# arendu-zz/MacaronicUserModeling

Hardware: AMD Instinct MI355X
Metric: LBP sweep iters/sec (whole node), batch=8192 graphs |X|=64 (higher is better)
Workload: dtype f64

## Files before the change

### macaronicusermodeling_amd/csrc/mlbp_lean.hip

```cpp
#include <hip/hip_runtime.h>

#include <vector>

#include "mlbp_device.h"
#include "mlbp_internal.h"

using mlbp::fail;
using namespace mlbp_dev;

namespace {

constexpr int WG = 256;

typedef double nt_d2 __attribute__((ext_vector_type(2)));
#define NT_LOAD2(p) ([&] { const nt_d2 v_ = __builtin_nontemporal_load(reinterpret_cast<const nt_d2*>(p)); return make_double2(v_.x, v_.y); }())

constexpr int UOP_VAR = 1;
constexpr int UOP_MT = 2;
constexpr int UOP_PSLOT_SHIFT = 2;
constexpr int UOP_NOP = 32;
constexpr int UOP_STORE_VF = 64;
constexpr int UOP_NSRC_SHIFT = 8;
constexpr int UOP_CARRY_IN = 0x1000;
constexpr int UOP_CARRY_OUT = 0x2000;
constexpr int GROUP_WORDS = 48;

struct LeanDev {
  const int32_t* image;
  const int32_t* readout;
  uint8_t* bail;
  int32_t n_bundles, HL, n_cprod, WL, n_ext, init, dense, keep;
};

__device__ __forceinline__ double swapadd16(double a, double b) {
  auto lo = __builtin_amdgcn_permlane16_swap((unsigned)__double2loint(a), (unsigned)__double2loint(b), false, false);
  auto hi = __builtin_amdgcn_permlane16_swap((unsigned)__double2hiint(a), (unsigned)__double2hiint(b), false, false);
  return __hiloint2double((int)hi[0], (int)lo[0]) + __hiloint2double((int)hi[1], (int)lo[1]);
}
__device__ __forceinline__ double swapadd32(double a, double b) {
  auto lo = __builtin_amdgcn_permlane32_swap((unsigned)__double2loint(a), (unsigned)__double2loint(b), false, false);
  auto hi = __builtin_amdgcn_permlane32_swap((unsigned)__double2hiint(a), (unsigned)__double2hiint(b), false, false);
  return __hiloint2double((int)hi[0], (int)lo[0]) + __hiloint2double((int)hi[1], (int)lo[1]);
}

__device__ __forceinline__ bool vote_any(bool p, int32_t* votes, int wave, int lane) {
  const int mine = __ballot(p) != 0 ? 1 : 0;
  if (lane == 0) votes[wave] = mine;
  lds_barrier();
  const int4 v = *reinterpret_cast<const int4*>(votes);
  return (v.x | v.y | v.z | v.w) != 0;
}

struct LaneGeo {
  int tm0, tm1;
  int mt;
  int red_tm;
  int red_mt;
  bool up, st_tm, st_mt, wr_tm;
};

__device__ __forceinline__ double2 lds2(const char* p) { return *reinterpret_cast<const double2*>(p); }
__device__ __forceinline__ void mul2(double2& a, const double2 b) { a.x *= b.x; a.y *= b.y; }

struct RegTable {
  const double2 (&T)[4][2];
  __device__ __forceinline__ double2 operator()(int r, int k) const { return T[r][k]; }
};
struct LdsTable {
  const double2* base;
  __device__ __forceinline__ double2 operator()(int r, int k) const { return base[(r * 2 + k) * WG]; }
};

template <bool MT, typename TB>
__device__ __forceinline__ void contract(const TB T, char* wb, int u0, int s1, int s2, int s3, int s4, int vf,
                                         const LaneGeo& G, char* redA) {
  const int nsrc = (u0 >> UOP_NSRC_SHIFT) & 15;
  const bool has_vf = (u0 & UOP_STORE_VF) != 0;
  if (MT) {
    double2 ma = lds2(wb + s1 + G.mt), mb = lds2(wb + s1 + G.mt + 16);
    if (nsrc > 1) {
      const double2 a = lds2(wb + s2 + G.mt), b = lds2(wb + s2 + G.mt + 16);
      mul2(ma, a); mul2(mb, b);
      if (nsrc > 2) {
        const double2 a2 = lds2(wb + s3 + G.mt), b2 = lds2(wb + s3 + G.mt + 16);
        mul2(ma, a2); mul2(mb, b2);
        if (nsrc > 3) { const double2 a3 = lds2(wb + s4 + G.mt), b3 = lds2(wb + s4 + G.mt + 16); mul2(ma, a3); mul2(mb, b3); }
      }
    }
    if (has_vf && G.st_mt) {
      *reinterpret_cast<double2*>(wb + vf + G.mt) = ma;
      *reinterpret_cast<double2*>(wb + vf + G.mt + 16) = mb;
    }
    double a00, a01, a10, a11;
    { const double2 t0 = T(0, 0), t1 = T(0, 1); a00 = ma.x * t0.x; a01 = ma.x * t0.y; a10 = ma.x * t1.x; a11 = ma.x * t1.y; }
    { const double2 t0 = T(1, 0), t1 = T(1, 1); a00 += ma.y * t0.x; a01 += ma.y * t0.y; a10 += ma.y * t1.x; a11 += ma.y * t1.y; }
    { const double2 t0 = T(2, 0), t1 = T(2, 1); a00 += mb.x * t0.x; a01 += mb.x * t0.y; a10 += mb.x * t1.x; a11 += mb.x * t1.y; }
    { const double2 t0 = T(3, 0), t1 = T(3, 1); a00 += mb.y * t0.x; a01 += mb.y * t0.y; a10 += mb.y * t1.x; a11 += mb.y * t1.y; }
    a00 += dpp_mov<0x128>(a10);
    a01 += dpp_mov<0x128>(a11);
    *reinterpret_cast<double*>(redA + G.red_mt) = swapadd32(a00, a01);
  } else {
    double2 m0 = lds2(wb + s1 + G.tm0), m1 = lds2(wb + s1 + G.tm1);
    if (nsrc > 1) {
      const double2 a = lds2(wb + s2 + G.tm0), b = lds2(wb + s2 + G.tm1);
      mul2(m0, a); mul2(m1, b);
      if (nsrc > 2) {
        const double2 a2 = lds2(wb + s3 + G.tm0), b2 = lds2(wb + s3 + G.tm1);
        mul2(m0, a2); mul2(m1, b2);
        if (nsrc > 3) { const double2 a3 = lds2(wb + s4 + G.tm0), b3 = lds2(wb + s4 + G.tm1); mul2(m0, a3); mul2(m1, b3); }
      }
    }
    if (has_vf && G.st_tm) {
      *reinterpret_cast<double2*>(wb + vf + G.tm0) = m0;
      *reinterpret_cast<double2*>(wb + vf + G.tm1) = m1;
    }
    double v[4];
#pragma unroll
    for (int r = 0; r < 4; ++r) {
      const double2 t0 = T(r, 0), t1 = T(r, 1);
      v[r] = t0.x * m0.x;
      v[r] += t0.y * m0.y;
      v[r] += t1.x * m1.x;
      v[r] += t1.y * m1.y;
    }
    const double u0 = swapadd16(v[0], v[2]), u1 = swapadd16(v[1], v[3]);
    const double keep = G.up ? u1 : u0, send = G.up ? u0 : u1;
    double w = keep + dpp_mov<0x141>(send);
    w += dpp_mov<0xB1>(w);
    w += dpp_mov<0x4E>(w);
    *reinterpret_cast<double*>(redA + G.red_tm) = w;
  }
}

template <int NT, int NL>
__device__ __forceinline__ void front(const double2 (&tab)[NT][4][2], const double2* tl, char* wb, int u0, const int4& lo, const int4& hi,
                                      const LaneGeo& G, char* redA) {
  const int pslot = (u0 >> UOP_PSLOT_SHIFT) & 7;
#pragma unroll
  for (int p = 0; p < NT; ++p) {
    if (p == pslot) {
      if (u0 & UOP_MT) contract<true>(RegTable{tab[p]}, wb, u0, lo.y, lo.z, lo.w, hi.x, hi.y, G, redA);
      else contract<false>(RegTable{tab[p]}, wb, u0, lo.y, lo.z, lo.w, hi.x, hi.y, G, redA);
    }
  }
  if (NL > 0 && pslot >= NT) {
    const LdsTable T = {tl + (size_t)(pslot - NT) * 8 * WG};
    if (u0 & UOP_MT) contract<true>(T, wb, u0, lo.y, lo.z, lo.w, hi.x, hi.y, G, redA);
    else contract<false>(T, wb, u0, lo.y, lo.z, lo.w, hi.x, hi.y, G, redA);
  }
}

template <int NT>
__device__ __forceinline__ void gradient_epilogue(const SweepDev& d, const GradFusedDev& gf, const double2 (&tab)[NT][4][2],
                                                  const char* wb, const int32_t* gst, double* scratch, const LaneGeo& G, int g,
                                                  int R_, int c_, int b3_) {
  constexpr int FEE = 3, FED = 6;
  const int t = threadIdx.x, lane = t & 63, wave = __builtin_amdgcn_readfirstlane(t >> 6);
  double lf[FEE] = {0.0, 0.0, 0.0};
  bool lbad = false;
  if (t < NT && t < d.P) {
    const int l0 = gf.pair_label[((size_t)g * d.P + t) * 2], l1 = gf.pair_label[((size_t)g * d.P + t) * 2 + 1];
    if ((unsigned)l0 >= 64u || (unsigned)l1 >= 64u) lbad = true;
    else {
      const double* phl = (gf.pair_phi[t] ? gf.phi_en_en_w1 : gf.phi_en_en) + ((size_t)l0 * 64 + l1) * FEE;
#pragma unroll
      for (int q = 0; q < FEE; ++q) lf[q] = phl[q];
    }
  }
  int which = 0;
  double2 W[NT][4][2];
  double* zs = scratch + 512;
  double* lfs = scratch + 544;
#pragma unroll
  for (int p = 0; p < NT; ++p) {
    double z = 0.0;
    if (p < d.P) {
      const int cs = as_const(gf.pair_c_slot)[p], rs = as_const(gf.pair_r_slot)[p];
      which |= (as_const(gf.pair_phi)[p] ? 1 : 0) << p;
      const double2 ca = lds2(wb + cs * 512 + G.mt), cb = lds2(wb + cs * 512 + G.mt + 16);
      const double2 r0 = lds2(wb + rs * 512 + G.tm0), r1 = lds2(wb + rs * 512 + G.tm1);
#pragma unroll
      for (int r = 0; r < 4; ++r) {
        const double ci = r == 0 ? ca.x : (r == 1 ? ca.y : (r == 2 ? cb.x : cb.y));
#pragma unroll
        for (int k = 0; k < 2; ++k) {
          const double2 rj = k ? r1 : r0, T = tab[p][r][k];
          W[p][r][k] = make_double2((ci * rj.x) * T.x, (ci * rj.y) * T.y);
          z += W[p][r][k].x + W[p][r][k].y;
        }
      }
      z = wave_sum(z);
      if (lane == 0) zs[wave * NT + p] = z;
    } else {
#pragma unroll
      for (int r = 0; r < 4; ++r) W[p][r][0] = W[p][r][1] = make_double2(0.0, 0.0);
    }
  }
  if (lbad) atomicExch(d.status, 1);
  if (t < NT && t < d.P) {
#pragma unroll
    for (int q = 0; q < FEE; ++q) lfs[t * FEE + q] = lf[q];
  }
  lds_barrier();
  double2 V[2][4][2];
#pragma unroll
  for (int tz = 0; tz < 2; ++tz)
#pragma unroll
    for (int r = 0; r < 4; ++r) V[tz][r][0] = V[tz][r][1] = make_double2(0.0, 0.0);
#pragma unroll
  for (int p = 0; p < NT; ++p) {
    if (p < d.P) {
      const double Z = (zs[p] + zs[NT + p]) + (zs[2 * NT + p] + zs[3 * NT + p]);
      const double inv = Z > 0.0 ? 1.0 / Z : 0.0;
      const double i0 = ((which >> p) & 1) ? 0.0 : inv, i1 = ((which >> p) & 1) ? inv : 0.0;
#pragma unroll
      for (int r = 0; r < 4; ++r)
#pragma unroll
        for (int k = 0; k < 2; ++k) {
          V[0][r][k].x += W[p][r][k].x * i0; V[0][r][k].y += W[p][r][k].y * i0;
          V[1][r][k].x += W[p][r][k].x * i1; V[1][r][k].y += W[p][r][k].y * i1;
        }
    }
  }
  double gacc[2][FEE] = {{0.0, 0.0, 0.0}, {0.0, 0.0, 0.0}};
  const int all = (1 << (d.P < NT ? d.P : NT)) - 1;
#pragma unroll
  for (int tz = 0; tz < 2; ++tz) {
    if (tz ? (which & all) == 0 : (which & all) == all) continue;
    typedef double v2d __attribute__((ext_vector_type(2)));
    typedef const v2d __attribute__((address_space(1))) * gptr2;
    const double* phi = tz ? gf.phi_en_en_w1 : gf.phi_en_en;
#pragma unroll
    for (int k = 0; k < 2; ++k) {
      const int col = 32 * (k ? 1 - b3_ : b3_) + 2 * c_;
      v2d cell[4][3];
#pragma unroll
      for (int r = 0; r < 4; ++r) {
        const gptr2 ph = (gptr2)(uintptr_t)(phi + ((size_t)(4 * R_ + r) * 64 + col) * FEE);
        cell[r][0] = ph[0]; cell[r][1] = ph[1]; cell[r][2] = ph[2];
      }
#pragma unroll
      for (int r = 0; r < 4; ++r) {
        const double w0 = V[tz][r][k].x, w1 = V[tz][r][k].y;
        gacc[tz][0] += w0 * cell[r][0].x + w1 * cell[r][1].y;
        gacc[tz][1] += w0 * cell[r][0].y + w1 * cell[r][2].x;
        gacc[tz][2] += w0 * cell[r][1].x + w1 * cell[r][2].y;
      }
    }
  }
  double gsum[FEE];
#pragma unroll
  for (int q = 0; q < FEE; ++q) gsum[q] = wave_sum(gacc[0][q] + gacc[1][q]);
  double lab_ee[FEE] = {0.0, 0.0, 0.0}, lab_ed[FED] = {0.0, 0.0, 0.0, 0.0, 0.0, 0.0};
  double exp_ee[FEE] = {0.0, 0.0, 0.0}, exp_ed[FED] = {0.0, 0.0, 0.0, 0.0, 0.0, 0.0};
  bool bad = false;
  constexpr int UB = 6;
  const int U = d.U;
  for (int u0 = wave; u0 < U; u0 += 4 * UB) {
    double b[UB], pv[UB][FED];
    int kd[UB], at[UB];
#pragma unroll
    for (int j = 0; j < UB; ++j) {
      const int u = u0 + 4 * j;
      kd[j] = -1;
      if (u < U) {
        const int kind = __builtin_amdgcn_readfirstlane(gst[2 * U + u]), obs = __builtin_amdgcn_readfirstlane(gst[3 * U + u]);
        const int lab = __builtin_amdgcn_readfirstlane(gst[4 * U + u]);
        const int cols = kind == 2 ? gf.Vde : 64;
        if ((unsigned)obs >= (unsigned)cols || (unsigned)lab >= 64u || (unsigned)kind > 2u) { bad = true; continue; }
        kd[j] = kind;
        const int slot = __builtin_amdgcn_readfirstlane(gst[u]);
        b[j] = __builtin_amdgcn_readfirstlane(gst[U + u]) ? *reinterpret_cast<const double*>(wb + slot * 512 + lane * 8) : 0.0;
        if (kind == 2) {
          const double2* ph = reinterpret_cast<const double2*>(gf.phi_en_de_t + ((size_t)obs * 64 + lane) * FED);
          at[j] = (obs * 64 + lab) * FED;
          const double2 a0 = ph[0], a1 = ph[1], a2 = ph[2];
          pv[j][0] = a0.x; pv[j][1] = a0.y; pv[j][2] = a1.x; pv[j][3] = a1.y; pv[j][4] = a2.x; pv[j][5] = a2.y;
        } else {
          typedef const double __attribute__((address_space(1))) * gptr1;
          const gptr1 ph = (gptr1)(uintptr_t)((kind ? gf.phi_en_en_w1_t : gf.phi_en_en_t) + ((size_t)obs * 64 + lane) * FEE);
          at[j] = (obs * 64 + lab) * FEE;
#pragma unroll
          for (int q = 0; q < FEE; ++q) pv[j][q] = ph[q];
        }
      }
    }
#pragma unroll
    for (int j = 0; j < UB; ++j) {
      if (kd[j] == 2) {
#pragma unroll
        for (int q = 0; q < FED; ++q) { lab_ed[q] += as_const_f64(gf.phi_en_de_t)[at[j] + q]; exp_ed[q] += b[j] * pv[j][q]; }
      } else if (kd[j] >= 0) {
        const double* base = kd[j] ? gf.phi_en_en_w1_t : gf.phi_en_en_t;
#pragma unroll
        for (int q = 0; q < FEE; ++q) { lab_ee[q] += as_const_f64(base)[at[j] + q]; exp_ee[q] += b[j] * pv[j][q]; }
      }
    }
  }
  if (bad && lane == 0) atomicExch(d.status, 1);
  constexpr int PER = FEE + FEE + FED;
  {
    double ue[FEE], ud[FED];
#pragma unroll
    for (int q = 0; q < FEE; ++q) ue[q] = lab_ee[q] - wave_sum(exp_ee[q]);
#pragma unroll
    for (int q = 0; q < FED; ++q) ud[q] = lab_ed[q] - wave_sum(exp_ed[q]);
    if (lane == 0) {
      double* o = scratch + wave * PER;
#pragma unroll
      for (int q = 0; q < FEE; ++q) o[q] = gsum[q];
#pragma unroll
      for (int q = 0; q < FEE; ++q) o[FEE + q] = ue[q];
#pragma unroll
      for (int q = 0; q < FED; ++q) o[FEE + FEE + q] = ud[q];
    }
  }
  lds_barrier();
  if (t == 0) {
    double tot[PER];
#pragma unroll
    for (int q = 0; q < PER; ++q) tot[q] = (scratch[q] + scratch[PER + q]) + (scratch[2 * PER + q] + scratch[3 * PER + q]);
    double gee[FEE];
#pragma unroll
    for (int q = 0; q < FEE; ++q) gee[q] = tot[FEE + q] - tot[q];
#pragma unroll
    for (int p = 0; p < NT; ++p) {
      if (p < d.P) {
#pragma unroll
        for (int q = 0; q < FEE; ++q) gee[q] += lfs[p * FEE + q];
      }
    }
#pragma unroll
    for (int q = 0; q < FEE; ++q) gf.grad_en_en[(size_t)g * FEE + q] = gee[q];
#pragma unroll
    for (int q = 0; q < FED; ++q) gf.grad_en_de[(size_t)g * FED + q] = tot[FEE + FEE + q];
  }
}

__device__ __forceinline__ double rescale(double r, int& bad) {
  const unsigned key = mag_key(r);
  const unsigned long long normal = __ballot(key - KEY_MIN < KEY_BAD - KEY_MIN);
  const unsigned long long wrong = __ballot(key >= KEY_BAD);
  bad |= (wrong != 0) | (normal == 0);
  const int ref = __builtin_amdgcn_readlane((int)key, normal ? __builtin_ctzll(normal) : 0);
  return __builtin_ldexp(r, 1023 - ((ref >> 20) & 0x7FF));
}

template <int NT, bool PADX, bool MULTI, int NL, bool GRAD>
__global__ __launch_bounds__(WG, (NT >= 7 ? 1 : (NT >= 4 ? 2 : 3))) void sweep_x64_lean_kernel(SweepDev d, LeanDev f, const int32_t* groups,
                                                                                             int n_groups, GradFusedDev gf) {
  int g = blockIdx.x;
  if (MULTI) {
    int lo = 0, hi = n_groups - 1;
    while (lo < hi) {
      const int mid = (lo + hi + 1) >> 1;
      if (as_const(groups)[(size_t)mid * GROUP_WORDS] <= g) lo = mid; else hi = mid - 1;
    }
    const int32_t* G = groups + (size_t)lo * GROUP_WORDS;
    const Words16 w0 = sload16(G), w1 = sload16(G + 16), w2 = sload16(G + 32);
    auto ptr = [](int32_t a, int32_t b) { return (uintptr_t)(uint32_t)a | ((uintptr_t)(uint32_t)b << 32); };
    g -= w0.w[0];
    f.image = (const int32_t*)ptr(w0.w[2], w0.w[3]); f.readout = (const int32_t*)ptr(w0.w[4], w0.w[5]);
    f.bail = (uint8_t*)ptr(w0.w[6], w0.w[7]); d.msgs = (double*)ptr(w0.w[8], w0.w[9]);
    d.marginals = (double*)ptr(w0.w[10], w0.w[11]); d.pair_tables = (const double*)ptr(w0.w[12], w0.w[13]);
    d.pair_tab = (const int32_t*)ptr(w0.w[14], w0.w[15]); d.unary_tables = (const double*)ptr(w1.w[0], w1.w[1]);
    d.unary_tab = (const int32_t*)ptr(w1.w[2], w1.w[3]); d.status = (int32_t*)ptr(w1.w[4], w1.w[5]);
    f.n_bundles = w1.w[6]; f.HL = w1.w[7]; f.n_cprod = w1.w[8]; f.WL = w1.w[9]; f.n_ext = w1.w[10];
    d.n_msgs = w1.w[11]; d.P = w1.w[12]; d.U = w1.w[13]; d.n_vars = w1.w[14]; d.n_pair_tables = w1.w[15];
    d.n_unary_tables = w2.w[0]; f.dense = w2.w[1];
  }
  extern __shared__ double lds[];
  double* work = lds;
  double* red = lds + (size_t)(d.n_msgs + f.n_ext) * 64;
  int32_t* limg = reinterpret_cast<int32_t*>(red + 4 * 256);
  double2* tl = reinterpret_cast<double2*>(limg + 16 * (f.n_bundles + 1));
  int32_t* gst = reinterpret_cast<int32_t*>(tl + (size_t)NL * 8 * WG);

  const int t = threadIdx.x, lane = t & 63, wave = __builtin_amdgcn_readfirstlane(t >> 6);
  const int X = PADX ? d.X : 64;
  const double uniform = 1.0 / (double)X;
  const double uni_l = (!PADX || lane < X) ? uniform : 0.0;
  double* gm = d.msgs + (size_t)g * d.n_msgs * X;
  const int32_t* img_hoist = f.image + 16 * (size_t)f.n_bundles;
  const int32_t* img_cprod = img_hoist + 8 * (size_t)f.HL;
  const int32_t* img_written = img_cprod + 16 * (size_t)f.n_cprod;
  int32_t* votes = reinterpret_cast<int32_t*>(red);
  constexpr bool LEAN_SYNC = !GRAD;

  LaneGeo G;
  const int c_ = (lane & 7) | ((lane >> 1) & 8), b3_ = (lane >> 3) & 1, R_ = 4 * wave + (b3_ | ((lane >> 5) << 1));
  {
    const int b5 = lane >> 5, b4 = (lane >> 4) & 1, b2 = (lane >> 2) & 1;
    G.tm0 = (32 * b3_ + 2 * c_) * 8;
    G.tm1 = (32 * (1 - b3_) + 2 * c_) * 8;
    G.mt = 4 * R_ * 8;
    G.red_tm = (4 * R_ + 2 * b4 + b2) * 8;
    G.red_mt = (wave * 64 + 32 * b3_ + 2 * c_ + b5) * 8;
    G.up = b2 != 0;
    G.st_tm = wave == 0 && (lane & 0x28) == 0;
    G.st_mt = (lane & 0x17) == 0;
    G.wr_tm = (lane & 3) == 0;
  }

  if (t == 0) f.bail[g] = 0;
  int g_kind = 0, g_obs = 0, g_lab = 0;
  if (GRAD && t < d.U) {
    g_kind = gf.unary_kind[t]; g_obs = gf.unary_obs[(size_t)g * d.U + t]; g_lab = gf.unary_label[(size_t)g * d.U + t];
  }
  bool ok = true;
  constexpr int HB = 8;
  double ur[HB];
  int uslot[HB], ufac[HB];
  {
    const Words16 hl = sload16(img_hoist + wave * 2 * f.HL);
#pragma unroll
    for (int j = 0; j < HB; ++j) {
      const int u = hl.w[2 * j];
      uslot[j] = hl.w[2 * j + 1];
      ufac[j] = u;
      ur[j] = 0.0;
      if (u >= 0) {
        const int row = f.dense ? g * d.U + u : as_const(d.unary_tab)[(size_t)g * d.U + u];
        if ((unsigned)row >= (unsigned)d.n_unary_tables) ok = false;
        else if (!PADX || lane < X) ur[j] = d.unary_tables[(size_t)row * X + lane];
      }
    }
  }
  double2 tab[NT][4][2];
#pragma unroll
  for (int p = 0; p < NT; ++p) {
    if (p < d.P) {
      const int ti = f.dense ? g * d.P + p : as_const(d.pair_tab)[(size_t)g * d.P + p];
      if ((unsigned)ti >= (unsigned)d.n_pair_tables) { ok = false; continue; }
      if (!PADX) {
        const double* T = d.pair_tables + (size_t)ti * 4096 + (size_t)(4 * R_) * 64 + 2 * c_;
#pragma unroll
        for (int r = 0; r < 4; ++r) {
          tab[p][r][0] = NT_LOAD2(T + r * 64 + 32 * b3_);
          tab[p][r][1] = NT_LOAD2(T + r * 64 + 32 * (1 - b3_));
        }
      } else {
        const double* T = d.pair_tables + (size_t)ti * X * X;
#pragma unroll
        for (int r = 0; r < 4; ++r)
#pragma unroll
          for (int k = 0; k < 2; ++k) {
            const int row = 4 * R_ + r, col = 32 * (k ? 1 - b3_ : b3_) + 2 * c_;
            tab[p][r][k].x = (row < X && col < X) ? T[(size_t)row * X + col] : 0.0;
            tab[p][r][k].y = (row < X && col + 1 < X) ? T[(size_t)row * X + col + 1] : 0.0;
          }
      }
    }
  }
#pragma unroll
  for (int p = NT; p < NT + NL; ++p) {
    if (p < d.P && !PADX) {
      const int ti = f.dense ? g * d.P + p : as_const(d.pair_tab)[(size_t)g * d.P + p];
      if ((unsigned)ti >= (unsigned)d.n_pair_tables) { ok = false; continue; }
      const double* T = d.pair_tables + (size_t)ti * 4096 + (size_t)(4 * R_) * 64 + 2 * c_;
#pragma unroll
      for (int r = 0; r < 4; ++r)
#pragma unroll
        for (int k = 0; k < 2; ++k) {
          typedef __attribute__((address_space(3))) void* lds_ptr;
          typedef const __attribute__((address_space(1))) void* glb_ptr;
          double2* dst = tl + ((p - NT) * 8 + r * 2 + k) * WG + wave * 64;
          __builtin_amdgcn_global_load_lds((glb_ptr)(T + r * 64 + 32 * (k ? 1 - b3_ : b3_)), (lds_ptr)dst, 16, 0, 0);
        }
    }
  }
  bool dense_ok = true;
  if (f.dense)
    for (int i = t; i < d.P + d.U; i += WG)
      dense_ok &= i < d.P ? d.pair_tab[(size_t)g * d.P + i] == g * d.P + i : d.unary_tab[(size_t)g * d.U + (i - d.P)] == g * d.U + (i - d.P);
  constexpr int PW = 2;
  int32_t pre[PW];
#pragma unroll
  for (int q = 0; q < PW; ++q) pre[q] = (t + q * WG < 16 * (f.n_bundles + 1)) ? f.image[t + q * WG] : 0;
  unsigned bad_key = 0;
  {
    double2* dst = reinterpret_cast<double2*>(work);
    const int x0 = (2 * t) & 63;
    const double2 uni2 = PADX ? make_double2(x0 < X ? uniform : 0.0, x0 + 1 < X ? uniform : 0.0) : make_double2(uniform, uniform);
    if (f.init) {
      for (int i = t; i < d.n_msgs * 32; i += WG) dst[i] = uni2;
    } else if (!PADX) {
      const double2* src = reinterpret_cast<const double2*>(gm);
      for (int i = t; i < d.n_msgs * 32; i += WG) {
        const double2 v = src[i];
        bad_key = max(bad_key, max(mag_key(v.x), mag_key(v.y)));
        dst[i] = v;
      }
    } else {
      for (int i = t; i < d.n_msgs * 64; i += WG) {
        const int slot = i >> 6, x = i & 63;
        const double v = x < X ? gm[(size_t)slot * X + x] : 0.0;
        bad_key = max(bad_key, mag_key(v));
        work[i] = v;
      }
    }
    if (t < 32) dst[d.n_msgs * 32 + t] = uni2;
    if (t >= 32 && t < 64) dst[(d.n_msgs + f.n_ext - 1) * 32 + (t - 32)] = make_double2(1.0, 1.0);
  }
  lds_barrier();
#pragma unroll
  for (int j = 0; j < HB; ++j) {
    if (uslot[j] >= 0) {
      const double s = wave_sum(ur[j]);
      const double m = renorm(ur[j], s, uni_l, true);
      bad_key = max(bad_key, s > 0.0 ? mag_key(m) : KEY_BAD);
      work[uslot[j] * 64 + lane] = m;
      if (GRAD && lane == 0) { gst[ufac[j]] = uslot[j]; gst[d.U + ufac[j]] = s > 0.0 ? 1 : 0; }
    }
  }
  if (GRAD && t < d.U) { gst[2 * d.U + t] = g_kind; gst[3 * d.U + t] = g_obs; gst[4 * d.U + t] = g_lab; }
  for (int j = HB; j < f.HL; ++j) {
    const const_i32p hp = as_const(img_hoist + (wave * f.HL + j) * 2);
    const int u = hp[0], slot = hp[1];
    if (u < 0) break;
    const int row = f.dense ? g * d.U + u : as_const(d.unary_tab)[(size_t)g * d.U + u];
    double r = 0.0;
    if ((unsigned)row >= (unsigned)d.n_unary_tables) ok = false;
    else if (!PADX || lane < X) r = d.unary_tables[(size_t)row * X + lane];
    const double s = wave_sum(r);
    const double m = renorm(r, s, uni_l, true);
    bad_key = max(bad_key, s > 0.0 ? mag_key(m) : KEY_BAD);
    work[slot * 64 + lane] = m;
    if (GRAD && lane == 0) { gst[u] = slot; gst[d.U + u] = s > 0.0 ? 1 : 0; }
  }
  if (LEAN_SYNC ? vote_any(!ok, votes, wave, lane) : !__syncthreads_and(ok ? 1 : 0)) {
    if (t == 0) atomicExch(d.status, 1);
    if (f.init)
      for (int i = t; i < d.n_msgs * X; i += WG) gm[i] = uniform;
    return;
  }
  for (int k = wave; k < f.n_cprod; k += 4) {
    const Words16 cl = sload16(img_cprod + 16 * k);
    double acc = uni_l;
#pragma unroll
    for (int q0 = 1; q0 < 16; q0 += 5) {
      if (cl.w[0] >= q0) {
        double m[5];
#pragma unroll
        for (int q = 0; q < 5; ++q) m[q] = work[cl.w[q0 + q] * 64 + lane];
#pragma unroll
        for (int q = 0; q < 5; ++q) acc *= m[q];
      }
    }
    bad_key = max(bad_key, mag_key(acc));
    work[(d.n_msgs + 1 + k) * 64 + lane] = acc;
  }
  auto fill_limg = [&]() {
    if (NL > 0) asm volatile("s_waitcnt vmcnt(0)" ::: "memory");
#pragma unroll
    for (int q = 0; q < PW; ++q)
      if (t + q * WG < 16 * (f.n_bundles + 1)) limg[t + q * WG] = pre[q];
    for (int i = t + PW * WG; i < 16 * (f.n_bundles + 1); i += WG) limg[i] = f.image[i];
  };
  if (LEAN_SYNC) fill_limg();
  if (LEAN_SYNC ? vote_any(bad_key >= KEY_BAD, votes + 1024, wave, lane) : __syncthreads_or(bad_key >= KEY_BAD ? 1 : 0) != 0) {
    if (t == 0) f.bail[g] = 1;
    return;
  }
  if (!LEAN_SYNC) { fill_limg(); lds_barrier(); }

  char* wb = reinterpret_cast<char*>(work);
  int parity = 0, bad = 0;
  double carry = 1.0;
  const int4* li = reinterpret_cast<const int4*>(limg);
  int4 A0 = li[0], A1 = li[1], B0 = li[2], B1 = li[3];
  for (int k = 0; k < f.n_bundles; ++k) {
    const int4 nA0 = li[4 * k + 4], nA1 = li[4 * k + 5], nB0 = li[4 * k + 6], nB1 = li[4 * k + 7];
    const int fA = __builtin_amdgcn_readfirstlane(A0.x), fB = __builtin_amdgcn_readfirstlane(B0.x);
    if (fA & UOP_VAR) {
      const int nsrc = (fA >> UOP_NSRC_SHIFT) & 15;
      double m = work[(A0.y >> 3) + lane];
      if (fA & UOP_CARRY_IN) m *= carry;
      if (nsrc > 1) m *= work[(A0.z >> 3) + lane];
      if (nsrc > 2) m *= work[(A0.w >> 3) + lane];
      if (nsrc > 3) m *= work[(A1.x >> 3) + lane];
      if (fA & UOP_CARRY_OUT) carry = m;
      else work[(A1.y >> 3) + lane] = m;
    } else {
      char* redP = reinterpret_cast<char*>(red) + parity * 4096;
      front<NT, NL>(tab, tl + t, wb, fA, A0, A1, G, redP);
      const bool two = !(fB & UOP_NOP);
      if (two) front<NT, NL>(tab, tl + t, wb, fB, B0, B1, G, redP + 2048);
      lds_barrier();
      const double* rd = reinterpret_cast<const double*>(redP);
      double rA = rd[lane];
      if (fA & UOP_MT) rA = (rA + rd[64 + lane]) + (rd[128 + lane] + rd[192 + lane]);
      work[(A1.z >> 3) + lane] = rescale(rA, bad);
      if (two) {
        double rB = rd[256 + lane];
        if (fB & UOP_MT) rB = (rB + rd[320 + lane]) + (rd[384 + lane] + rd[448 + lane]);
        work[(B1.z >> 3) + lane] = rescale(rB, bad);
      }
      parity ^= 1;
    }
    A0 = nA0; A1 = nA1; B0 = nB0; B1 = nB1;
  }
  if (bad) {
    if (t == 0) f.bail[g] = 2;
    return;
  }
  lds_barrier();
  double marg[2] = {0.0, 0.0};
  bool bad_out = !dense_ok;
  if (f.readout) {
#pragma unroll
    for (int j = 0; j < 2; ++j) {
      const int v = wave + 4 * j;
      if (v < d.n_vars) {
        const Words16 rl = sload16(f.readout + 16 * v);
        double acc = work[rl.w[1] * 64 + lane];
#pragma unroll
        for (int q0 = 2; q0 < 16; q0 += 7) {
          if (rl.w[0] >= q0) {
            double m[7];
#pragma unroll
            for (int q = 0; q < 7; ++q) m[q] = work[rl.w[q0 + q] * 64 + lane];
#pragma unroll
            for (int q = 0; q < 7; ++q) acc *= m[q];
          }
        }
        const unsigned key = wave_max_u32(mag_key(acc));
        bad_out |= key >= KEY_BAD || key < KEY_MIN;
        marg[j] = acc / wave_sum(acc);
      }
    }
    for (int v = wave + 8; v < d.n_vars; v += 4) {
      const Words16 rl = sload16(f.readout + 16 * v);
      double acc = work[rl.w[1] * 64 + lane];
      for (int q = 2; q <= rl.w[0]; ++q) acc *= work[as_const(f.readout + 16 * v)[q] * 64 + lane];
      const unsigned key = wave_max_u32(mag_key(acc));
      bad_out |= key >= KEY_BAD || key < KEY_MIN;
      if (!bad_out) d.marginals[((size_t)g * d.n_vars + v) * 64 + lane] = acc / wave_sum(acc);
    }
  }
  lds_barrier();
  if (f.keep || GRAD) {
    for (int j0 = 0; j0 < f.WL; j0 += 4) {
      const const_i32p wl = as_const(img_written + wave * f.WL + j0);
      int slot[4];
      double v[4], s[4];
#pragma unroll
      for (int j = 0; j < 4; ++j) { slot[j] = wl[j]; v[j] = slot[j] >= 0 ? work[slot[j] * 64 + lane] : 1.0; }
#pragma unroll
      for (int j = 0; j < 4; ++j) {
        const unsigned key = wave_max_u32(mag_key(v[j]));
        bad_out |= key >= KEY_BAD || key < KEY_MIN;
        s[j] = wave_sum(v[j]);
      }
#pragma unroll
      for (int j = 0; j < 4; ++j)
        if (slot[j] >= 0) work[slot[j] * 64 + lane] = v[j] / s[j];
    }
  }
  if (LEAN_SYNC ? vote_any(bad_out, votes, wave, lane) : __syncthreads_or(bad_out ? 1 : 0) != 0) {
    if (t == 0) f.bail[g] = 3;
    return;
  }
  if (f.keep && !PADX) {
    const double2* src = reinterpret_cast<const double2*>(work);
    double2* dst = reinterpret_cast<double2*>(gm);
    for (int i = t; i < d.n_msgs * 32; i += WG) dst[i] = src[i];
  } else if (f.keep) {
    for (int i = t; i < d.n_msgs * 64; i += WG)
      if ((i & 63) < X) gm[(size_t)(i >> 6) * X + (i & 63)] = work[i];
  }
  if (f.readout) {
#pragma unroll
    for (int j = 0; j < 2; ++j) {
      const int v = wave + 4 * j;
      if (v < d.n_vars) d.marginals[((size_t)g * d.n_vars + v) * 64 + lane] = marg[j];
    }
  }
  if (GRAD) {
    gradient_epilogue<NT>(d, gf, tab, reinterpret_cast<const char*>(work), gst, reinterpret_cast<double*>(red), G, g, R_, c_, b3_);
  }
}

}

namespace mlbp {

void build_lean_program(const FusedProgram& fp, int n_msgs, LeanProgram& out) {
  out = LeanProgram();
  if (fp.has_unary_fops) { out.why = "in-loop unary updates (not hoistable)"; return; }
  std::vector<int32_t> U;
  std::vector<char> second;
  auto emit_var = [&](const int32_t* src, int n, int c) {
    int done = 0;
    do {
      int32_t w[8] = {0, 0, 0, 0, 0, 0, 0, 0};
      int k = 0;
      const bool first = done == 0;
      while (k < 4 && done < n) w[1 + k++] = src[done++] * 512;
      w[0] = UOP_VAR | (k << UOP_NSRC_SHIFT) | (first ? 0 : UOP_CARRY_IN) | (done < n ? UOP_CARRY_OUT : 0);
      w[5] = c * 512;
      U.insert(U.end(), w, w + 8);
      second.push_back(0);
    } while (done < n);
  };
  const int n_fops = (int)fp.fops.size() / 8;
  for (int i = 0; i < n_fops; ++i) {
    const int32_t* w = &fp.fops[8 * (size_t)i];
    const int kind = w[0] & 0xFF;
    if (kind == FOP_VAR) { emit_var(&fp.psrcs[w[1]], w[2], w[3]); continue; }
    const int members = (w[0] & FOP_BUNDLED) ? 2 : 1;
    for (int m = 0; m < members; ++m) {
      const int32_t* q = &fp.fops[8 * (size_t)(i + m)];
      const int kd = q[0] & 0xFF;
      if ((kd == FOP_VAR_PAIR_TM || kd == FOP_VAR_PAIR_MT) && q[2] > 4) emit_var(&fp.psrcs[q[1]], q[2], q[3]);
    }
    for (int m = 0; m < members; ++m) {
      const int32_t* q = &fp.fops[8 * (size_t)(i + m)];
      const int kd = q[0] & 0xFF;
      int32_t u[8] = {0, 0, 0, 0, 0, -1, 0, 0};
      if (kd == FOP_PAIR_TM || kd == FOP_PAIR_MT) {
        u[0] = (kd == FOP_PAIR_MT ? UOP_MT : 0) | (q[1] << UOP_PSLOT_SHIFT) | (1 << UOP_NSRC_SHIFT);
        u[1] = q[2] * 512;
        u[6] = q[3] * 512;
      } else {
        const bool chained = q[2] > 4;
        const int n = chained ? 1 : q[2];
        u[0] = (kd == FOP_VAR_PAIR_MT ? UOP_MT : 0) | (q[4] << UOP_PSLOT_SHIFT) | (n << UOP_NSRC_SHIFT);
        if (chained) u[1] = q[3] * 512;
        else for (int k = 0; k < n; ++k) u[1 + k] = fp.psrcs[q[1] + k] * 512;
        u[5] = chained ? -1 : q[3] * 512;
        u[6] = q[5] * 512;
      }
      U.insert(U.end(), u, u + 8);
      second.push_back(m == 1);
    }
    i += members - 1;
  }
  const int n_uops = (int)U.size() / 8;
  for (int i = 0; i < n_uops; ++i) {
    int32_t* u = &U[8 * (size_t)i];
    if ((u[0] & UOP_VAR) || u[5] < 0) continue;
    const int c = u[5];
    bool needed = true;
    for (int j = i + 1; j < n_uops; ++j) {
      const int32_t* v = &U[8 * (size_t)j];
      const int n = (v[0] >> UOP_NSRC_SHIFT) & 15;
      bool reads = false;
      for (int k = 0; k < n; ++k) reads |= v[1 + k] == c;
      if (reads) break;
      const bool writes = v[5] == c || (!(v[0] & UOP_VAR) && v[6] == c);
      if (writes) { needed = false; break; }
    }
    if (!needed) u[5] = -1;
  }
  for (int i = 0; i < n_uops; ++i) {
    int32_t* u = &U[8 * (size_t)i];
    if (!(u[0] & UOP_VAR) && u[5] >= 0) u[0] |= UOP_STORE_VF;
    if (u[5] < 0) u[5] = 0;
  }
  std::vector<int32_t>& I = out.image;
  const int32_t nop[8] = {UOP_NOP, 0, 0, 0, 0, -1, 0, 0};
  for (int i = 0; i < n_uops; ++i) {
    I.insert(I.end(), U.begin() + 8 * (size_t)i, U.begin() + 8 * (size_t)i + 8);
    if (i + 1 < n_uops && second[i + 1]) { ++i; I.insert(I.end(), U.begin() + 8 * (size_t)i, U.begin() + 8 * (size_t)i + 8); }
    else I.insert(I.end(), nop, nop + 8);
  }
  out.n_bundles = (int)I.size() / 16;
  const int n_hoist = (int)fp.hoist.size() / 2;
  out.HL = std::max(8, ((n_hoist + 3) / 4 + 7) / 8 * 8);
  {
    std::vector<int32_t> hl(4 * (size_t)out.HL * 2, -1);
    for (int h = 0; h < n_hoist; ++h) {
      hl[((size_t)(h & 3) * out.HL + (h >> 2)) * 2] = fp.hoist[2 * h];
      hl[((size_t)(h & 3) * out.HL + (h >> 2)) * 2 + 1] = fp.hoist[2 * h + 1];
    }
    I.insert(I.end(), hl.begin(), hl.end());
  }
  out.n_cprod = fp.n_cprod;
  const int ones = n_msgs + 1 + fp.n_cprod;
  out.cprods.clear();
  for (size_t at = 0; at < fp.cpw.size();) {
    const int cnt = fp.cpw[at];
    if (cnt > 15) { out.why = "a constant product of more than 15 messages"; out.image.clear(); return; }
    int32_t l[16];
    l[0] = cnt;
    for (int q = 0; q < 15; ++q) l[1 + q] = q < cnt ? fp.cpw[at + 1 + q] : ones;
    I.insert(I.end(), l, l + 16);
    out.cprods.push_back(std::vector<int32_t>(fp.cpw.begin() + at + 1, fp.cpw.begin() + at + 1 + cnt));
    at += 1 + cnt;
  }
  out.hoisted.assign(n_msgs, 0);
  for (int h = 0; h < n_hoist; ++h) out.hoisted[fp.hoist[2 * h + 1]] = 1;
  const int n_written = (int)fp.written.size();
  out.WL = std::max(4, ((n_written + 3) / 4 + 3) / 4 * 4);
  {
    std::vector<int32_t> wl(4 * (size_t)out.WL, -1);
    for (int i = 0; i < n_written; ++i) wl[(size_t)(i & 3) * out.WL + (i >> 2)] = fp.written[i];
    I.insert(I.end(), wl.begin(), wl.end());
  }
  for (int q = 0; q < 16; ++q) I.push_back(q == 0 || q == 8 ? UOP_NOP : 0);
  out.ok = true;
}

bool build_lean_readout(const LeanProgram& lp, int n_msgs, int n_vars, const int32_t* in_off, const int32_t* in_slots,
                        std::vector<int32_t>& image) {
  image.assign(16 * (size_t)n_vars, n_msgs);
  for (int v = 0; v < n_vars; ++v) {
    std::vector<int32_t> consts, vars;
    for (int q = in_off[v]; q < in_off[v + 1]; ++q) (lp.hoisted[in_slots[q]] ? consts : vars).push_back(in_slots[q]);
    int base = n_msgs;
    if (!consts.empty()) {
      size_t k = 0;
      for (; k < lp.cprods.size(); ++k)
        if (lp.cprods[k] == consts) break;
      if (k < lp.cprods.size()) base = n_msgs + 1 + (int)k;
      else { vars.insert(vars.begin(), consts.begin(), consts.end()); }
    }
    if (vars.size() > 14) return false;
    int32_t* l = &image[16 * (size_t)v];
    l[0] = 1 + (int)vars.size();
    l[1] = base;
    const int ones = n_msgs + 1 + lp.n_cprod;
    for (int q = 0; q < 14; ++q) l[2 + q] = q < (int)vars.size() ? vars[q] : ones;
  }
  return true;
}

static int lean_plan(const mlbp_program* prog, const mlbp_sweep_args* a, bool grad, bool* ok, SweepDev* d, LeanDev* f, size_t* lds) {
  *ok = false;
  const LeanProgram& lp = prog->lean;
  if (!lp.ok || !prog->d_limage || a->X > 64 || a->X < 2 || !a->normalize_messages || prog->P < 1 || prog->P > 8) return MLBP_OK;
  const bool padx = a->X < 64;
  if (padx && prog->P > 4) return MLBP_OK;
  if (a->gradient && padx) return MLBP_OK;
  if (grad && (prog->P > 3 || prog->U > WG)) return fail(MLBP_EINVAL, "lean kernel: fused gradient needs P <= 3 and U <= %d", WG);
  if (a->flags & MLBP_SWEEP_APPROX_INFERENCE) return MLBP_OK;
  if (a->marginals && !prog->d_lreadout && !padx) return MLBP_OK;
  const int n_ext = 2 + lp.n_cprod;
  *lds = ((size_t)(prog->n_msgs + n_ext) * 64 + 4 * 256) * sizeof(double) + 16 * (size_t)(lp.n_bundles + 1) * sizeof(int32_t);
  if (prog->P == 7 && !padx) *lds += 32 * 1024;
  if (grad) *lds += 5 * (size_t)prog->U * sizeof(int32_t);
  if (*lds > 80 * 1024) return MLBP_OK;
  const bool dense = (a->flags & MLBP_SWEEP_DENSE_TABLES) != 0;
  if (dense && ((int64_t)a->B * prog->P > a->n_pair_tables || (int64_t)a->B * prog->U > a->n_unary_tables))
    return fail(MLBP_EINVAL, "mlbp_sweep_f64: MLBP_SWEEP_DENSE_TABLES needs B*P pair tables and B*U unary columns");
  mlbp_program* mp = const_cast<mlbp_program*>(prog);
  if (mp->bail_cap < a->B)
    if (int e = mlbp_program_reserve(mp, a->B)) return e;
  d->pair_tables = a->pair_tables; d->pair_tab = a->pair_tab;
  d->unary_tables = a->unary_tables; d->unary_tab = a->unary_tab;
  d->msgs = a->msgs;
  d->ops = nullptr; d->srcs = nullptr; d->sweeps = nullptr; d->pairseq = nullptr;
  d->status = prog->d_status;
  d->n_sweeps = prog->n_sweeps; d->n_msgs = prog->n_msgs; d->P = prog->P; d->U = prog->U; d->X = a->X;
  d->n_pair_tables = a->n_pair_tables; d->n_unary_tables = a->n_unary_tables;
  d->marginals = padx ? nullptr : a->marginals; d->readout = nullptr; d->n_vars = prog->n_vars;
  d->only = nullptr; d->fill_uniform = 0; d->approx_k = 0;
  f->image = prog->d_limage; f->readout = (a->marginals && !padx) ? prog->d_lreadout : nullptr; f->bail = mp->d_bail;
  f->n_bundles = lp.n_bundles; f->HL = lp.HL; f->n_cprod = lp.n_cprod; f->WL = lp.WL;
  f->n_ext = n_ext; f->init = a->init_messages; f->dense = dense ? 1 : 0;
  const bool waived = (a->flags & MLBP_SWEEP_NO_MESSAGE_WRITEBACK) && !padx && (a->marginals || grad) && (!a->gradient || grad);
  f->keep = waived ? 0 : 1;
  *ok = true;
  return MLBP_OK;
}

typedef void (*lean_fn)(SweepDev, LeanDev, const int32_t*, int, GradFusedDev);

template <bool MULTI>
static lean_fn pick_lean(int P, bool padx) {
  if constexpr (!MULTI) {
    if (padx) {
      switch (P) {
        case 1: return sweep_x64_lean_kernel<1, true, false, 0, false>;
        case 2: return sweep_x64_lean_kernel<2, true, false, 0, false>;
        case 3: return sweep_x64_lean_kernel<3, true, false, 0, false>;
        default: return sweep_x64_lean_kernel<4, true, false, 0, false>;
      }
    }
  }
  switch (P) {
    case 1: return sweep_x64_lean_kernel<1, false, MULTI, 0, false>;
    case 2: return sweep_x64_lean_kernel<2, false, MULTI, 0, false>;
    case 3: return sweep_x64_lean_kernel<3, false, MULTI, 0, false>;
    case 4: return sweep_x64_lean_kernel<4, false, MULTI, 0, false>;
    case 5: case 6: return sweep_x64_lean_kernel<6, false, MULTI, 0, false>;
    case 7: return sweep_x64_lean_kernel<6, false, MULTI, 1, false>;
    default: return sweep_x64_lean_kernel<8, false, MULTI, 0, false>;
  }
}
static lean_fn pick_lean_grad(int P) {
  switch (P) {
    case 1: return sweep_x64_lean_kernel<1, false, false, 0, true>;
    case 2: return sweep_x64_lean_kernel<2, false, false, 0, true>;
    default: return sweep_x64_lean_kernel<3, false, false, 0, true>;
  }
}

int launch_lean_sweep(const mlbp_program* prog, const mlbp_sweep_args* a, const GradFusedDev* gf, void* stream, bool* launched) {
  *launched = false;
  SweepDev d;
  LeanDev f;
  size_t lds = 0;
  bool ok = false;
  if (int e = lean_plan(prog, a, gf != nullptr, &ok, &d, &f, &lds)) return e;
  if (!ok) return MLBP_OK;
  lean_fn k = gf ? pick_lean_grad(prog->P) : pick_lean<false>(prog->P, a->X < 64);
  if (int e = grant_lds((const void*)k, lds)) return e;
  launch_begin();
  MLBP_LAUNCH(k, dim3(a->B), dim3(WG), lds, (hipStream_t)stream, d, f, nullptr, 0, gf ? *gf : GradFusedDev{});
  if (int e = launch_verdict("lean sweep")) return e;
  *launched = true;
  return MLBP_OK;
}

int launch_lean_groups(const mlbp_program* const* progs, const mlbp_sweep_args* args, int n_groups, void* stream, std::vector<char>& member) {
  std::vector<int32_t> table;
  size_t lds_max = 0;
  int p_max = 0, total = 0, n_in = 0;
  SweepDev d0;
  LeanDev f0;
  for (int k = 0; k < n_groups; ++k) {
    if (!member[k]) continue;
    member[k] = 0;
    if (args[k].X != 64) continue;
    SweepDev d;
    LeanDev f;
    size_t lds = 0;
    bool ok = false;
    if (int e = lean_plan(progs[k], &args[k], false, &ok, &d, &f, &lds)) return e;
    if (!ok) continue;
    if (n_in == 0) { d0 = d; f0 = f; }
    else if (f.init != f0.init || f.keep != f0.keep || (f.readout != nullptr) != (f0.readout != nullptr)) continue;
    member[k] = 1;
    ++n_in;
    lds_max = std::max(lds_max, lds + (progs[k]->P < 7 ? 32 * 1024 : 0));
    p_max = std::max(p_max, (int)progs[k]->P);
    table.resize(table.size() + GROUP_WORDS, 0);
    int32_t* w = &table[table.size() - GROUP_WORDS];
    auto put = [&](int at, const void* p) { const uintptr_t v = (uintptr_t)p; w[at] = (int32_t)(uint32_t)v; w[at + 1] = (int32_t)(uint32_t)(v >> 32); };
    w[0] = total; w[1] = args[k].B;
    put(2, f.image); put(4, f.readout); put(6, f.bail); put(8, d.msgs); put(10, d.marginals); put(12, d.pair_tables);
    put(14, d.pair_tab); put(16, d.unary_tables); put(18, d.unary_tab); put(20, d.status);
    w[22] = f.n_bundles; w[23] = f.HL; w[24] = f.n_cprod; w[25] = f.WL; w[26] = f.n_ext; w[27] = d.n_msgs; w[28] = d.P; w[29] = d.U;
    w[30] = d.n_vars; w[31] = d.n_pair_tables; w[32] = d.n_unary_tables; w[33] = f.dense;
    total += args[k].B;
  }
  if (n_in == 0) return MLBP_OK;
  mlbp_program* owner = const_cast<mlbp_program*>(progs[0]);
  int32_t* d_gtable = nullptr;
  if (int e = group_table_device(owner->gtables, table, stream, &d_gtable)) return e;
  lean_fn k = pick_lean<true>(p_max, false);
  if (int e = grant_lds((const void*)k, lds_max)) return e;
  launch_begin();
  MLBP_LAUNCH(k, dim3(total), dim3(WG), lds_max, (hipStream_t)stream, d0, f0, d_gtable, n_in, GradFusedDev{});
  return launch_verdict("grouped lean sweep");
}

}
```

Before: 13120.

## Make prologue loads and message-product reads branch-free with padded source slots

```diff
diff --git a/macaronicusermodeling_amd/csrc/mlbp_lean.hip b/macaronicusermodeling_amd/csrc/mlbp_lean.hip
--- a/macaronicusermodeling_amd/csrc/mlbp_lean.hip
+++ b/macaronicusermodeling_amd/csrc/mlbp_lean.hip
@@ -71,20 +71,26 @@
   __device__ __forceinline__ double2 operator()(int r, int k) const { return base[(r * 2 + k) * WG]; }
 };
 
-template <bool MT, typename TB>
+template <bool MT, bool WIDE, typename TB>
 __device__ __forceinline__ void contract(const TB T, char* wb, int u0, int s1, int s2, int s3, int s4, int vf,
                                          const LaneGeo& G, char* redA) {
   const int nsrc = (u0 >> UOP_NSRC_SHIFT) & 15;
   const bool has_vf = (u0 & UOP_STORE_VF) != 0;
   if (MT) {
     double2 ma = lds2(wb + s1 + G.mt), mb = lds2(wb + s1 + G.mt + 16);
-    if (nsrc > 1) {
+    {
       const double2 a = lds2(wb + s2 + G.mt), b = lds2(wb + s2 + G.mt + 16);
       mul2(ma, a); mul2(mb, b);
-      if (nsrc > 2) {
+    }
+    if (nsrc > 2) {
+      if (WIDE) {
         const double2 a2 = lds2(wb + s3 + G.mt), b2 = lds2(wb + s3 + G.mt + 16);
+        const double2 a3 = lds2(wb + s4 + G.mt), b3 = lds2(wb + s4 + G.mt + 16);
         mul2(ma, a2); mul2(mb, b2);
-        if (nsrc > 3) { const double2 a3 = lds2(wb + s4 + G.mt), b3 = lds2(wb + s4 + G.mt + 16); mul2(ma, a3); mul2(mb, b3); }
+        mul2(ma, a3); mul2(mb, b3);
+      } else {
+        mul2(ma, lds2(wb + s3 + G.mt)); mul2(mb, lds2(wb + s3 + G.mt + 16));
+        if (nsrc > 3) { mul2(ma, lds2(wb + s4 + G.mt)); mul2(mb, lds2(wb + s4 + G.mt + 16)); }
       }
     }
     if (has_vf && G.st_mt) {
@@ -101,13 +107,19 @@
     *reinterpret_cast<double*>(redA + G.red_mt) = swapadd32(a00, a01);
   } else {
     double2 m0 = lds2(wb + s1 + G.tm0), m1 = lds2(wb + s1 + G.tm1);
-    if (nsrc > 1) {
+    {
       const double2 a = lds2(wb + s2 + G.tm0), b = lds2(wb + s2 + G.tm1);
       mul2(m0, a); mul2(m1, b);
-      if (nsrc > 2) {
+    }
+    if (nsrc > 2) {
+      if (WIDE) {
         const double2 a2 = lds2(wb + s3 + G.tm0), b2 = lds2(wb + s3 + G.tm1);
+        const double2 a3 = lds2(wb + s4 + G.tm0), b3 = lds2(wb + s4 + G.tm1);
         mul2(m0, a2); mul2(m1, b2);
-        if (nsrc > 3) { const double2 a3 = lds2(wb + s4 + G.tm0), b3 = lds2(wb + s4 + G.tm1); mul2(m0, a3); mul2(m1, b3); }
+        mul2(m0, a3); mul2(m1, b3);
+      } else {
+        mul2(m0, lds2(wb + s3 + G.tm0)); mul2(m1, lds2(wb + s3 + G.tm1));
+        if (nsrc > 3) { mul2(m0, lds2(wb + s4 + G.tm0)); mul2(m1, lds2(wb + s4 + G.tm1)); }
       }
     }
     if (has_vf && G.st_tm) {
@@ -139,14 +151,14 @@
 #pragma unroll
   for (int p = 0; p < NT; ++p) {
     if (p == pslot) {
-      if (u0 & UOP_MT) contract<true>(RegTable{tab[p]}, wb, u0, lo.y, lo.z, lo.w, hi.x, hi.y, G, redA);
-      else contract<false>(RegTable{tab[p]}, wb, u0, lo.y, lo.z, lo.w, hi.x, hi.y, G, redA);
+      if (u0 & UOP_MT) contract<true, (NT > 1)>(RegTable{tab[p]}, wb, u0, lo.y, lo.z, lo.w, hi.x, hi.y, G, redA);
+      else contract<false, (NT > 1)>(RegTable{tab[p]}, wb, u0, lo.y, lo.z, lo.w, hi.x, hi.y, G, redA);
     }
   }
   if (NL > 0 && pslot >= NT) {
     const LdsTable T = {tl + (size_t)(pslot - NT) * 8 * WG};
-    if (u0 & UOP_MT) contract<true>(T, wb, u0, lo.y, lo.z, lo.w, hi.x, hi.y, G, redA);
-    else contract<false>(T, wb, u0, lo.y, lo.z, lo.w, hi.x, hi.y, G, redA);
+    if (u0 & UOP_MT) contract<true, (NT > 1)>(T, wb, u0, lo.y, lo.z, lo.w, hi.x, hi.y, G, redA);
+    else contract<false, (NT > 1)>(T, wb, u0, lo.y, lo.z, lo.w, hi.x, hi.y, G, redA);
   }
 }
 
@@ -386,6 +398,8 @@
   const int32_t* img_written = img_cprod + 16 * (size_t)f.n_cprod;
   int32_t* votes = reinterpret_cast<int32_t*>(red);
   constexpr bool LEAN_SYNC = !GRAD;
+  constexpr bool EARLY = !GRAD;
+  static_assert(!(GRAD && PADX), "the GRAD form of phase A loads whole rows: X = 64 only");
 
   LaneGeo G;
   const int c_ = (lane & 7) | ((lane >> 1) & 8), b3_ = (lane >> 3) & 1, R_ = 4 * wave + (b3_ | ((lane >> 5) << 1));
@@ -408,6 +422,7 @@
     g_kind = gf.unary_kind[t]; g_obs = gf.unary_obs[(size_t)g * d.U + t]; g_lab = gf.unary_label[(size_t)g * d.U + t];
   }
   bool ok = true;
+  const double* nowhere = reinterpret_cast<const double*>(f.image);
   constexpr int HB = 8;
   double ur[HB];
   int uslot[HB], ufac[HB];
@@ -418,18 +433,38 @@
       const int u = hl.w[2 * j];
       uslot[j] = hl.w[2 * j + 1];
       ufac[j] = u;
-      ur[j] = 0.0;
-      if (u >= 0) {
-        const int row = f.dense ? g * d.U + u : as_const(d.unary_tab)[(size_t)g * d.U + u];
-        if ((unsigned)row >= (unsigned)d.n_unary_tables) ok = false;
-        else if (!PADX || lane < X) ur[j] = d.unary_tables[(size_t)row * X + lane];
+      if (EARLY) {
+        int row = -1;
+        if (u >= 0) row = f.dense ? g * d.U + u : as_const(d.unary_tab)[(size_t)g * d.U + u];
+        const bool in = (unsigned)row < (unsigned)d.n_unary_tables;
+        if (u >= 0 && !in) ok = false;
+        const double* at = in ? d.unary_tables + (size_t)row * X + (PADX ? min(lane, X - 1) : lane) : nowhere;
+        ur[j] = *at;
+      } else {
+        ur[j] = 0.0;
+        if (u >= 0) {
+          const int row = f.dense ? g * d.U + u : as_const(d.unary_tab)[(size_t)g * d.U + u];
+          if ((unsigned)row >= (unsigned)d.n_unary_tables) ok = false;
+          else ur[j] = d.unary_tables[(size_t)row * X + lane];
+        }
       }
     }
   }
   double2 tab[NT][4][2];
 #pragma unroll
   for (int p = 0; p < NT; ++p) {
-    if (p < d.P) {
+    if (!PADX && EARLY) {
+      const int pc = p < d.P ? p : 0;
+      const int ti = f.dense ? g * d.P + pc : as_const(d.pair_tab)[(size_t)g * d.P + pc];
+      const bool in = (unsigned)ti < (unsigned)d.n_pair_tables;
+      if (p < d.P && !in) ok = false;
+      const double* T = (p < d.P && in) ? d.pair_tables + (size_t)ti * 4096 + (size_t)(4 * R_) * 64 + 2 * c_ : nowhere;
+#pragma unroll
+      for (int r = 0; r < 4; ++r) {
+        tab[p][r][0] = NT_LOAD2(T + r * 64 + 32 * b3_);
+        tab[p][r][1] = NT_LOAD2(T + r * 64 + 32 * (1 - b3_));
+      }
+    } else if (p < d.P) {
       const int ti = f.dense ? g * d.P + p : as_const(d.pair_tab)[(size_t)g * d.P + p];
       if ((unsigned)ti >= (unsigned)d.n_pair_tables) { ok = false; continue; }
       if (!PADX) {
@@ -469,14 +504,21 @@
         }
     }
   }
+  int dense_word = 0;
   bool dense_ok = true;
-  if (f.dense)
+  if (EARLY) {
+    const int i = min(t, d.P + d.U - 1);
+    const int32_t* at = i < d.P ? d.pair_tab + (size_t)g * d.P + i : d.unary_tab + (size_t)g * d.U + (i - d.P);
+    dense_word = *(f.dense ? at : f.image);
+  } else if (f.dense) {
     for (int i = t; i < d.P + d.U; i += WG)
       dense_ok &= i < d.P ? d.pair_tab[(size_t)g * d.P + i] == g * d.P + i : d.unary_tab[(size_t)g * d.U + (i - d.P)] == g * d.U + (i - d.P);
+  }
   constexpr int PW = 2;
   int32_t pre[PW];
 #pragma unroll
-  for (int q = 0; q < PW; ++q) pre[q] = (t + q * WG < 16 * (f.n_bundles + 1)) ? f.image[t + q * WG] : 0;
+  for (int q = 0; q < PW; ++q)
+    pre[q] = EARLY ? f.image[min(t + q * WG, 16 * (f.n_bundles + 1) - 1)] : ((t + q * WG < 16 * (f.n_bundles + 1)) ? f.image[t + q * WG] : 0);
   unsigned bad_key = 0;
   {
     double2* dst = reinterpret_cast<double2*>(work);
@@ -506,8 +548,9 @@
 #pragma unroll
   for (int j = 0; j < HB; ++j) {
     if (uslot[j] >= 0) {
-      const double s = wave_sum(ur[j]);
-      const double m = renorm(ur[j], s, uni_l, true);
+      const double r = (!PADX || lane < X) ? ur[j] : 0.0;
+      const double s = wave_sum(r);
+      const double m = renorm(r, s, uni_l, true);
       bad_key = max(bad_key, s > 0.0 ? mag_key(m) : KEY_BAD);
       work[uslot[j] * 64 + lane] = m;
       if (GRAD && lane == 0) { gst[ufac[j]] = uslot[j]; gst[d.U + ufac[j]] = s > 0.0 ? 1 : 0; }
@@ -575,10 +618,14 @@
     if (fA & UOP_VAR) {
       const int nsrc = (fA >> UOP_NSRC_SHIFT) & 15;
       double m = work[(A0.y >> 3) + lane];
+      const double m2 = work[(A0.z >> 3) + lane];
       if (fA & UOP_CARRY_IN) m *= carry;
-      if (nsrc > 1) m *= work[(A0.z >> 3) + lane];
-      if (nsrc > 2) m *= work[(A0.w >> 3) + lane];
-      if (nsrc > 3) m *= work[(A1.x >> 3) + lane];
+      m *= m2;
+      if (nsrc > 2) {
+        const double m3 = work[(A0.w >> 3) + lane], m4 = work[(A1.x >> 3) + lane];
+        m *= m3;
+        m *= m4;
+      }
       if (fA & UOP_CARRY_OUT) carry = m;
       else work[(A1.y >> 3) + lane] = m;
     } else {
@@ -606,6 +653,7 @@
   }
   lds_barrier();
   double marg[2] = {0.0, 0.0};
+  if (EARLY) dense_ok = !f.dense || t >= d.P + d.U || dense_word == (t < d.P ? g * d.P + t : g * d.U + (t - d.P));
   bool bad_out = !dense_ok;
   if (f.readout) {
 #pragma unroll
@@ -689,11 +737,12 @@
   out = LeanProgram();
   if (fp.has_unary_fops) { out.why = "in-loop unary updates (not hoistable)"; return; }
   std::vector<int32_t> U;
+  const int32_t ones = (n_msgs + 1 + fp.n_cprod) * 512;
   std::vector<char> second;
   auto emit_var = [&](const int32_t* src, int n, int c) {
     int done = 0;
     do {
-      int32_t w[8] = {0, 0, 0, 0, 0, 0, 0, 0};
+      int32_t w[8] = {0, ones, ones, ones, ones, 0, 0, 0};
       int k = 0;
       const bool first = done == 0;
       while (k < 4 && done < n) w[1 + k++] = src[done++] * 512;
@@ -717,7 +766,7 @@
     for (int m = 0; m < members; ++m) {
       const int32_t* q = &fp.fops[8 * (size_t)(i + m)];
       const int kd = q[0] & 0xFF;
-      int32_t u[8] = {0, 0, 0, 0, 0, -1, 0, 0};
+      int32_t u[8] = {0, ones, ones, ones, ones, -1, 0, 0};
       if (kd == FOP_PAIR_TM || kd == FOP_PAIR_MT) {
         u[0] = (kd == FOP_PAIR_MT ? UOP_MT : 0) | (q[1] << UOP_PSLOT_SHIFT) | (1 << UOP_NSRC_SHIFT);
         u[1] = q[2] * 512;
@@ -777,14 +826,13 @@
     I.insert(I.end(), hl.begin(), hl.end());
   }
   out.n_cprod = fp.n_cprod;
-  const int ones = n_msgs + 1 + fp.n_cprod;
   out.cprods.clear();
   for (size_t at = 0; at < fp.cpw.size();) {
     const int cnt = fp.cpw[at];
     if (cnt > 15) { out.why = "a constant product of more than 15 messages"; out.image.clear(); return; }
     int32_t l[16];
     l[0] = cnt;
-    for (int q = 0; q < 15; ++q) l[1 + q] = q < cnt ? fp.cpw[at + 1 + q] : ones;
+    for (int q = 0; q < 15; ++q) l[1 + q] = q < cnt ? fp.cpw[at + 1 + q] : ones / 512;
     I.insert(I.end(), l, l + 16);
     out.cprods.push_back(std::vector<int32_t>(fp.cpw.begin() + at + 1, fp.cpw.begin() + at + 1 + cnt));
     at += 1 + cnt;
@@ -799,6 +847,7 @@
     I.insert(I.end(), wl.begin(), wl.end());
   }
   for (int q = 0; q < 16; ++q) I.push_back(q == 0 || q == 8 ? UOP_NOP : 0);
+  if (I.size() < 512) I.resize(512, 0);
   out.ok = true;
 }
 
@@ -841,6 +890,7 @@
   if (prog->P == 7 && !padx) *lds += 32 * 1024;
   if (grad) *lds += 5 * (size_t)prog->U * sizeof(int32_t);
   if (*lds > 80 * 1024) return MLBP_OK;
+  if (prog->P + prog->U > WG) return MLBP_OK;
   const bool dense = (a->flags & MLBP_SWEEP_DENSE_TABLES) != 0;
   if (dense && ((int64_t)a->B * prog->P > a->n_pair_tables || (int64_t)a->B * prog->U > a->n_unary_tables))
     return fail(MLBP_EINVAL, "mlbp_sweep_f64: MLBP_SWEEP_DENSE_TABLES needs B*P pair tables and B*U unary columns");
```

Result: faster. 13740, median of 6 (+4.7%).
